# hasindu2008/cornetto

Hardware: AMD Instinct MI355X
Metric: Gbases/s scanned (telowin+sdust+boringbits) (higher is better)
Workload: dtype u8/u16 integer

## Files before the change

### cornetto_amd/csrc/sdust_sift.hpp

```cpp
#pragma once

struct SiftArgs {
    const uint8_t *bases;
    const int64_t *ctg_off;
    const int32_t *ctg_len;
    const SdChunk *chunks;
    int32_t n_chunks;
    int32_t T, W;
    uint32_t lds_per_wave;
    uint32_t reg_cap;
    const uint32_t *order;
    uint32_t *walk_out;
    uint32_t *iswalk_out;
    uint32_t *counter;
    int32_t thr, lmin;
    int32_t abl;
    int32_t dp_min;
    int32_t l2_skip;
};

#ifndef SIFT_WPB
#define SIFT_WPB 1
#endif
constexpr int SIFT_NCTR = 64;
constexpr int SIFT_PAD = 16;
#ifndef SIFT_K
#define SIFT_K 16
#endif
constexpr int SIFT_LS = SIFT_K - 1;
constexpr int SIFT_FIXED = 1024 + 512;
__host__ __device__ constexpr uint32_t sift_lds_bytes(uint32_t cap) { return (SIFT_FIXED + cap / 4 + 2 * (SIFT_PAD + cap) + 16 + 15) / 16 * 16; }


__device__ __forceinline__ uint32_t sd_codes4(uint32_t word)
{
    const uint32_t y = word & 0xDFDFDFDFu, idx = y & 0x07070707u;
    const uint32_t code = __builtin_amdgcn_perm(0x02000003u, 0x01000000u, idx);
    const uint32_t d = y ^ __builtin_amdgcn_perm(0x47FFFF54u, 0x43FF41FFu, idx);
    const uint32_t nz = ((d & 0x7F7F7F7Fu) + 0x7F7F7F7Fu) | d;
    return code | ((nz >> 5) & 0x04040404u);
}
__device__ __forceinline__ uint32_t sd_words4(uint32_t cn, uint32_t pcn)
{
    const uint32_t y1 = __builtin_amdgcn_alignbyte(cn, pcn, 3);
    const uint32_t y2 = __builtin_amdgcn_alignbyte(cn, pcn, 2);
    const uint32_t t = (cn & 0x03030303u) | ((y1 & 0x03030303u) << 2) | ((y2 & 0x03030303u) << 4);
    return t | (((cn | y1 | y2) & 0x04040404u) << 4);
}

__device__ __forceinline__ int sd_mbcnt64(unsigned long long m)
{
    return (int)__builtin_amdgcn_mbcnt_hi((uint32_t)(m >> 32), __builtin_amdgcn_mbcnt_lo((uint32_t)m, 0u));
}
__device__ __forceinline__ int sd_dpp_shr1(int old, int src, bool zero_fill)
{
    return zero_fill ? __builtin_amdgcn_update_dpp(0, src, 0x138, 0xF, 0xF, true) : __builtin_amdgcn_update_dpp(old, src, 0x138, 0xF, 0xF, false);
}

__device__ const uint32_t sd_recip_tab[64] = {0x0u, 0x0u, 0x80000000u, 0x55555556u, 0x40000000u, 0x33333334u, 0x2AAAAAABu, 0x24924925u, 0x20000000u, 0x1C71C71Du, 0x1999999Au, 0x1745D175u, 0x15555556u, 0x13B13B14u, 0x12492493u, 0x11111112u, 0x10000000u, 0xF0F0F10u, 0xE38E38Fu, 0xD79435Fu, 0xCCCCCCDu, 0xC30C30Du, 0xBA2E8BBu, 0xB21642Du, 0xAAAAAABu, 0xA3D70A4u, 0x9D89D8Au, 0x97B425Fu, 0x924924Au, 0x8D3DCB1u, 0x8888889u, 0x8421085u, 0x8000000u, 0x7C1F07Du, 0x7878788u, 0x7507508u, 0x71C71C8u, 0x6EB3E46u, 0x6BCA1B0u, 0x6906907u, 0x6666667u, 0x63E7064u, 0x6186187u, 0x5F417D1u, 0x5D1745Eu, 0x5B05B06u, 0x590B217u, 0x572620Bu, 0x5555556u, 0x539782Au, 0x51EB852u, 0x5050506u, 0x4EC4EC5u, 0x4D4873Fu, 0x4BDA130u, 0x4A7904Bu, 0x4924925u, 0x47DC120u, 0x469EE59u, 0x456C798u, 0x4444445u, 0x4325C54u, 0x4210843u, 0x4104105u};

__device__ __forceinline__ uint32_t sd_scan_max_dpp(uint32_t x)
{
    asm volatile("s_nop 1\n\t"
                 "v_max_u32_dpp %0, %0, %0 row_shr:1 row_mask:0xf bank_mask:0xf\n\ts_nop 1\n\t"
                 "v_max_u32_dpp %0, %0, %0 row_shr:2 row_mask:0xf bank_mask:0xf\n\ts_nop 1\n\t"
                 "v_max_u32_dpp %0, %0, %0 row_shr:4 row_mask:0xf bank_mask:0xf\n\ts_nop 1\n\t"
                 "v_max_u32_dpp %0, %0, %0 row_shr:8 row_mask:0xf bank_mask:0xf\n\ts_nop 1\n\t"
                 "v_max_u32_dpp %0, %0, %0 row_bcast:15 row_mask:0xa bank_mask:0xf\n\ts_nop 1\n\t"
                 "v_max_u32_dpp %0, %0, %0 row_bcast:31 row_mask:0xc bank_mask:0xf\n\ts_nop 1"
                 : "+v"(x));
    return x;
}

__device__ __forceinline__ int sd_wave_find_start(const SdChunk ch, const uint8_t *seq, int W, int lane)
{
    if (ch.start <= 0) return 0;
    const int y = ch.start - 2 * W;
    if (y <= 2) return 0;
    int need = W - 2;
    for (int tile = (y - 1) >> 6, it = 0; tile >= 0 && it < 64; --tile, ++it) {
        const int p = tile * 64 + lane;
        const bool isb = p < y && nt4_code(seq[p]) < 4;
        const unsigned long long b = sd_ballot(isb);
        need -= __popcll(b & (b << 1) & (b << 2));
        if (need <= 0 || tile == 0) return tile * 64;
    }
    return -2;
}

#ifndef SIFT_CHUNK_DEFAULT
#define SIFT_CHUNK_DEFAULT 1792
#endif
constexpr uint32_t SIFT_CAP_DEFAULT = SIFT_CHUNK_DEFAULT + 128;
template <bool STATS, uint32_t CAP = 0>
__global__ __launch_bounds__(64 * SIFT_WPB) __attribute__((amdgpu_waves_per_eu(CAP ? 7 : 6))) void sd_sift(SiftArgs A, SdArgs O)
{
    extern __shared__ __attribute__((aligned(16))) uint8_t sift_lds[];
    const int lane = threadIdx.x & 63;
    const int wave = SIFT_WPB == 1 ? 0 : __builtin_amdgcn_readfirstlane((int)(threadIdx.x >> 6));
    uint8_t *const L = sift_lds + (size_t)wave * (CAP ? sift_lds_bytes(CAP) : A.lds_per_wave);
    uint32_t *const tab = reinterpret_cast<uint32_t *>(L);
    uint16_t *const tl = reinterpret_cast<uint16_t *>(L + 1024);
    uint16_t *const tl2 = tl + 128;
    uint32_t *const sb = reinterpret_cast<uint32_t *>(L + SIFT_FIXED);
    const uint32_t cap = CAP ? CAP : A.reg_cap;
#ifdef CN_DEV
    const int abl = CAP ? 0 : A.abl;
#else
    constexpr int abl = 0;
#endif
    constexpr int STAGE_ROUNDS = CAP ? (int)((CAP + 1023) / 1024) : 4;
    uint32_t *const cb = sb + (cap >> 5);
    uint4 *const col = reinterpret_cast<uint4 *>(tab);
    uint8_t *const wc = L + SIFT_FIXED + cap / 4 + 2 * SIFT_PAD;
    const int T = A.T, W = A.W, CAPW = W - 2;

    const int lo = lane - (CAPW - 1);
    const unsigned long long below = lane ? ~0ull >> (64 - lane) : 0ull;
    const unsigned long long mc = lo > 0 ? below & (~0ull << lo) : below;
    const unsigned long long mp = lo < 0 ? ~0ull << (64 + lo) : 0ull;
    const uint32_t m_a = (uint32_t)mc, m_d = (uint32_t)(mp >> 32), m_m = lane < 32 ? (uint32_t)mp : (uint32_t)(mc >> 32);
    const uint32_t mybit = 1u << (lane & 31);
    uint32_t *const mine0 = tab + (lane < 32 ? 0 : 192), *const mine1 = tab + (lane < 32 ? 64 : 128);
    uint32_t *const tab_mine = mine0;
    const uint32_t *const mid1 = tab + (lane < 32 ? 0 : 128);
    const int thr = A.thr, lmin = A.lmin;
    const int LS = CAPW - 1 < SIFT_LS ? CAPW - 1 : SIFT_LS;
    const bool long_ok = CAPW - 1 > LS;
    unsigned long long st_steps = 0, st_jumps = 0, st_cand = 0, st_trig = 0, st_l1 = 0, st_l2 = 0, st_walk = 0, st_tiles = 0, st_dp = 0, st_g2 = 0, st_g4 = 0, st_g8 = 0;

    struct Meta {
        SdChunk ch;
        int len;
        const uint8_t *seq;
    };
    struct Data {
        uint4 q[2];
        uint32_t pw[2];
    };
    auto meta = [&](int kk) {
        Meta m;
        m.ch = A.chunks[kk];
        m.len = A.ctg_len[m.ch.ctg];
        m.seq = A.bases + A.ctg_off[m.ch.ctg];
        return m;
    };
    auto fetch = [&](const Meta &m) {
        Data d;
        const int rb = m.ch.start - (m.ch.start > 0 ? 128 : 0), rlen = m.ch.end - rb;
#pragma unroll
        for (int it = 0; it < 2; ++it) {
            const int b16 = lane * 16 + it * 1024;
            d.q[it] = make_uint4(0, 0, 0, 0);
            if (b16 < rlen) d.q[it] = *reinterpret_cast<const uint4 *>(m.seq + rb + b16);
        }
        uint32_t first = 0;
        if (rb > 0) first = *reinterpret_cast<const uint32_t *>(m.seq + rb - 4);
        d.pw[0] = (uint32_t)__builtin_amdgcn_update_dpp((int)first, (int)d.q[0].w, 0x138, 0xF, 0xF, false);
        d.pw[1] = (uint32_t)__builtin_amdgcn_update_dpp(rdlane((int)d.q[0].w, 63), (int)d.q[1].w, 0x138, 0xF, 0xF, false);
        return d;
    };

  auto process = [&](const int k, const Meta &M, const Data &D) {
    const SdChunk ch = M.ch;
    const int len = M.len;
    const uint8_t *seq = M.seq;
    const int halo = ch.start > 0 ? 128 : 0;
    const int rb = ch.start - halo;
    const int rlen = ch.end - rb;
    const int ntile = (rlen + 63) >> 6;
    const bool islast = ch.end == len;
    const int rec_from = ch.start;

    tab[lane] = 0;
    tab[64 + lane] = 0;
    tab[128 + lane] = 0;
    tab[192 + lane] = 0;
    for (int i = lane; i < (int)(cap >> 4); i += 64) sb[i] = 0;
    if (lane < SIFT_PAD) reinterpret_cast<uint16_t *>(wc)[lane - SIFT_PAD] = halo ? 0xFF40 : 0x0040;
    bool bad = false;
    bool general = rb <= 0 || rb + ((rlen + 15) & ~15) > len || (abl & 32);
    if (abl & 128) general = false;
    if (!general && !(abl & 128)) {
        uint32_t acc = 0u;
        int lane_s = lane * 16;
        for (int b16 = lane * 16, it = 0; it < STAGE_ROUNDS && b16 < rlen; b16 += 1024, ++it) {
            uint4 q;
            uint32_t pw;
            if (STAGE_ROUNDS <= 2 || it < 2) {
                q = D.q[it];
                pw = D.pw[it];
            } else {
                asm volatile("" : "+v"(lane_s));
                const uint8_t *const g = seq + rb + lane_s + it * 1024;
                q = *reinterpret_cast<const uint4 *>(g);
                pw = *reinterpret_cast<const uint32_t *>(g - 4);
            }
            const uint32_t ipw = pw & 0x07070707u;
            uint32_t pcn = __builtin_amdgcn_perm(0x02000003u, 0x01000000u, ipw);
            acc |= (pw & 0xDFDFDFDFu) ^ __builtin_amdgcn_perm(0x47FFFF54u, 0x43FF41FFu, ipw);
            const uint32_t in[4] = {q.x, q.y, q.z, q.w};
            uint32_t wo[8];
#pragma unroll
            for (int d = 0; d < 4; ++d) {
                const uint32_t idx = in[d] & 0x07070707u;
                const uint32_t cn = __builtin_amdgcn_perm(0x02000003u, 0x01000000u, idx);
                acc |= (in[d] & 0xDFDFDFDFu) ^ __builtin_amdgcn_perm(0x47FFFF54u, 0x43FF41FFu, idx);
                const uint32_t y1 = __builtin_amdgcn_alignbyte(cn, pcn, 3), y2 = __builtin_amdgcn_alignbyte(cn, pcn, 2);
                const uint32_t w4 = cn | y1 << 2 | y2 << 4;
                wo[2 * d] = __builtin_amdgcn_perm(0u, w4, 0x0C010C00u);
                wo[2 * d + 1] = __builtin_amdgcn_perm(0u, w4, 0x0C030C02u);
                pcn = cn;
            }
            uint4 *dst = reinterpret_cast<uint4 *>(wc + 2 * b16);
            dst[0] = make_uint4(wo[0], wo[1], wo[2], wo[3]);
            dst[1] = make_uint4(wo[4], wo[5], wo[6], wo[7]);
        }
        general = sd_any(acc != 0u);
    }
    if (general)
    for (int b16 = lane * 16, it = 0; it < STAGE_ROUNDS && b16 < rlen; b16 += 1024, ++it) {
        const int p0 = rb + b16;
        uint4 q;
        uint32_t pw;
        if (STAGE_ROUNDS <= 2 || it < 2) {
            q = D.q[it];
            pw = D.pw[it];
        } else {
            q = *reinterpret_cast<const uint4 *>(seq + p0);
            pw = *reinterpret_cast<const uint32_t *>(seq + p0 - 4);
        }
        uint32_t pcn = 0x04040404u;
        if (p0 > 0) pcn = sd_codes4(pw);
        const uint32_t in[4] = {q.x, q.y, q.z, q.w};
        uint32_t wo[8];
#pragma unroll
        for (int d = 0; d < 4; ++d) {
            uint32_t cn = sd_codes4(in[d]);
            if (p0 + 4 * d + 4 > len) {
                const int rem = len - (p0 + 4 * d);
                const uint32_t beyond = rem <= 0 ? 0xFFFFFFFFu : 0xFFFFFFFFu << (8 * rem);
                bad = bad || (cn & 0x04040404u & ~beyond) != 0u;
                cn |= 0x04040404u & beyond;
            } else {
                bad = bad || (cn & 0x04040404u) != 0u;
            }
            const uint32_t w4 = sd_words4(cn, pcn);
            wo[2 * d] = __builtin_amdgcn_perm(0u, w4, 0x0C010C00u);
            wo[2 * d + 1] = __builtin_amdgcn_perm(0u, w4, 0x0C030C02u);
            pcn = cn;
        }
        uint4 *dst = reinterpret_cast<uint4 *>(wc + 2 * b16);
        dst[0] = make_uint4(wo[0], wo[1], wo[2], wo[3]);
        dst[1] = make_uint4(wo[4], wo[5], wo[6], wo[7]);
    }
    const bool unclean = sd_any(bad);
    SD_LDS_ORDER();

    int w = 0, r = 0, slot = 0;
    int sv0 = 0;
    bool have_last = false;
    uint32_t last_s = 0, last_f = 0, n_out = 0;
    uint2 *const out = O.out + (size_t)k * O.cap;
    auto emit = [&](int ps, int pf, int tm) {
        if (tm < rec_from) return;
        if (have_last && ps <= (int)last_f) {
            if (pf > (int)last_f) last_f = (uint32_t)pf;
        } else {
            if (have_last) {
                if (n_out < O.cap && lane == 0) out[n_out] = make_uint2(last_s, last_f);
                ++n_out;
            }
            have_last = true;
            last_s = (uint32_t)ps;
            last_f = (uint32_t)pf;
        }
    };
    auto emit_slots = [&](int from, int tm) {
        unsigned long long em = sd_ballot(slot != 0 && lane >= from && lane < CAPW);
        while (em) {
            const int a = 63 - __builtin_clzll(em);
            em &= ~(1ull << a);
            const uint32_t so = (uint32_t)rdlane(slot, a);
            const int s = sv0 - a;
            emit(s, s + (int)(so >> 24) + 3, tm);
        }
    };
    auto push_word = [&](int tw, int amax, bool age_slots) {
        const unsigned long long e = sd_ballot(w == tw) & ~(~1ull << (amax - 1 < 0 ? 0 : amax - 1)) & (amax > 0 ? ~0ull : 0ull);
        r = sd_dpp_shr1(0, r, true) + sd_mbcnt64(e);
        w = sd_dpp_shr1(tw, w, false);
        if (age_slots) slot = sd_dpp_shr1(0, slot, true);
    };
    auto pass = [&](int amax, const int Tl, const uint32_t m_recip) {
        const unsigned long long cm = sd_ballot(__mul24(r, 10) > Tl) & ~(~1ull << amax) & ~1ull;
        if (cm) {
            const bool cand = (cm >> lane) & 1ull;
            if (STATS) ++st_cand;
            uint32_t key_c = 0u;
            if (cand) key_c = lane == 1 ? ((uint32_t)r & 0x7FFu) << 13 : __umulhi(((uint32_t)r & 0x7FFu) << 13, m_recip);
            const uint32_t key_e = (uint32_t)slot & 0xFFFFFFu;
            const uint32_t xs = sd_scan_max_dpp(key_e > key_c ? key_e : key_c);
            const uint32_t sk = (uint32_t)__builtin_amdgcn_update_dpp(0, (int)xs, 0x138, 0xF, 0xF, true);
            const uint32_t km = sk > key_e ? sk : key_e;
            if (cand && key_c >= km) slot = (int)(key_c | ((uint32_t)lane << 24));
        }
    };
    auto finish = [&]() {
        if (have_last) {
            if (n_out < O.cap && lane == 0) out[n_out] = make_uint2(last_s, last_f);
            ++n_out;
        }
        if (lane == 0) {
            O.out_n[k] = n_out;
            if (n_out > O.cap) atomicMax(O.ovf, n_out);
            if (STATS) st_tiles += (unsigned long long)ntile;
        }
    };

    if (unclean) {
        const int Tl = T * lane;
        const uint32_t m_recip = sd_recip_tab[lane];
        if (A.walk_out && lane == 0) {
            A.iswalk_out[k] = 1u;
            A.walk_out[2 + atomicAdd(&A.walk_out[0], 1u)] = (uint32_t)k;
        }
        int u = sd_wave_find_start(ch, seq, W, lane);
        if (u == -2) u = __builtin_amdgcn_readfirstlane(sd_find_start<true>(O, ch, seq));
        if (u < 0) return;
        const int stop = islast ? len + 1 : ch.end;
        int l = 0, size = 0, cv = 4, ctile = -1;
        unsigned t = 0;
        for (int i = u; i < stop; ++i) {
            if ((i >> 6) != ctile) {
                ctile = i >> 6;
                const int p = ctile * 64 + lane;
                cv = p < len ? nt4_code(seq[p]) : 4;
            }
            const int b = rdlane(cv, i & 63);
            if (STATS) ++st_walk;
            if (b < 4) {
                ++l;
                t = (t << 2 | (unsigned)b) & 63u;
                if (l >= 3) {
                    const int start = (l - W > 0 ? l - W : 0) + (i + 1 - l);
                    const bool full = size >= CAPW;
                    const bool moves = l > W;
                    if (full && moves) {
                        const uint32_t so = (uint32_t)rdlane(slot, CAPW - 1);
                        if (so) {
                            const int s = sv0 - (CAPW - 1);
                            emit(s, s + (int)(so >> 24) + 3, i);
                        }
                    }
                    size = full ? CAPW : size + 1;
                    push_word((int)t, size - 1, !full || moves);
                    sv0 = start + size - 1;
                    pass(size - 1, Tl, m_recip);
                }
            } else {
                emit_slots(0, i);
                slot = 0;
                l = 0;
                t = 0;
            }
        }
        finish();
        return;
    }

    typedef __attribute__((address_space(3))) uint32_t lds_u32;
    int ntl = 0, ntl2 = 0;
#ifdef SIFT_L2_ADAPT
    int l2_hot = 0, l2_skipped = 0;
#endif
    auto run_l2 = [&](int nb) {
        const bool on = lane < nb;
        const int o = on ? (int)tl2[lane] : 0;
        bool keep = on;
        if (LS == SIFT_LS) {
            const uint32_t at = (uint32_t)(uintptr_t)(lds_u32 *)wc + 2u * (uint32_t)o - 2u * (uint32_t)(SIFT_K - 1);
            const lds_u32 *const pa = (const lds_u32 *)(uintptr_t)(at & ~3u);
            const uint32_t sh = at & 3u;
            uint32_t k80, ksel1, ksel2, ksel3, kw, kc;
            asm volatile("s_mov_b32 %0, 0x3f3f3f3f\n\ts_mov_b32 %1, 0x01010101\n\ts_mov_b32 %2, 0x02020202\n\ts_mov_b32 %3, 0x03030303\n\t"
                         "s_mov_b32 %4, 0x06040200\n\ts_mov_b32 %5, 0x07050301"
                         : "=s"(k80), "=s"(ksel1), "=s"(ksel2), "=s"(ksel3), "=s"(kw), "=s"(kc));
            uint32_t tt = (uint32_t)T;
            asm volatile("" : "+s"(tt));
            uint32_t Q[4];
#pragma unroll
            for (int q = 0; q < 4; ++q) {
                const uint32_t d0 = pa[2 * q], d1 = pa[2 * q + 1], d2 = pa[2 * q + 2];
                Q[q] = __builtin_amdgcn_perm(__builtin_amdgcn_alignbyte(d2, d1, sh), __builtin_amdgcn_alignbyte(d1, d0, sh), kc);
            }
            uint32_t S = 0;
            unsigned long long pos_m = ~0ull;
#pragma unroll
            for (int a = 0; a < SIFT_K; ++a) {
                const int idx = SIFT_K - 1 - a;
                switch (idx & 3) {
                case 0: asm("v_add_u32_sdwa %0, %1, %0 dst_sel:DWORD dst_unused:UNUSED_PAD src0_sel:BYTE_0 src1_sel:DWORD" : "+v"(S) : "v"(Q[idx >> 2])); break;
                case 1: asm("v_add_u32_sdwa %0, %1, %0 dst_sel:DWORD dst_unused:UNUSED_PAD src0_sel:BYTE_1 src1_sel:DWORD" : "+v"(S) : "v"(Q[idx >> 2])); break;
                case 2: asm("v_add_u32_sdwa %0, %1, %0 dst_sel:DWORD dst_unused:UNUSED_PAD src0_sel:BYTE_2 src1_sel:DWORD" : "+v"(S) : "v"(Q[idx >> 2])); break;
                default: asm("v_add_u32_sdwa %0, %1, %0 dst_sel:DWORD dst_unused:UNUSED_PAD src0_sel:BYTE_3 src1_sel:DWORD" : "+v"(S) : "v"(Q[idx >> 2])); break;
                }
                const uint32_t th = (tt * (uint32_t)(a + 1)) / 10u;
                unsigned long long ok = __builtin_amdgcn_ballot_w64(S > th);
                asm volatile("" : "+s"(ok), "+v"(S));
                pos_m &= ok;
            }
            uint32_t at2 = at & ~3u;
            asm volatile("" : "+v"(at2), "+s"(pos_m));
            const lds_u32 *const pb = (const lds_u32 *)(uintptr_t)at2;
            uint32_t P[4];
#pragma unroll
            for (int q = 0; q < 4; ++q) {
                const uint32_t d0 = pb[2 * q], d1 = pb[2 * q + 1], d2 = pb[2 * q + 2];
                P[q] = __builtin_amdgcn_perm(__builtin_amdgcn_alignbyte(d2, d1, sh), __builtin_amdgcn_alignbyte(d1, d0, sh), kw);
            }
            const uint32_t seen = (P[0] | P[1] | P[2] | P[3]) & 0xC0C0C0C0u;
            uint32_t ne = 0;
            unsigned long long sc_m = 0ull;
#pragma unroll
            for (int a = 1; a < SIFT_K; ++a) {
                const int idx = SIFT_K - 1 - a, qi = idx >> 2, bj = idx & 3;
                const uint32_t rep = __builtin_amdgcn_perm(P[qi], P[qi], bj == 0 ? 0u : bj == 1 ? ksel1 : bj == 2 ? ksel2 : ksel3);
#pragma unroll
                for (int q = qi; q < 4; ++q) {
                    if (q == qi && bj == 3) continue;
                    const uint32_t m = q == qi ? 0x40404040u << (8 * (bj + 1)) : 0x40404040u;
                    const uint32_t u = (P[q] ^ rep) + k80;
                    ne += (uint32_t)__builtin_popcount(u & m);
                }
                const int lim = a * (a + 1) / 2 - (int)((tt * (uint32_t)a) / 10u);
                unsigned long long hit = __builtin_amdgcn_ballot_w64((int)ne < lim);
                asm volatile("" : "+s"(hit), "+v"(ne), "+v"(P[0]), "+v"(P[1]), "+v"(P[2]), "+v"(P[3]));
                sc_m |= hit;
            }
            const bool sc = (sc_m >> lane) & 1ull, pos = (pos_m >> lane) & 1ull;
            keep = on && (seen != 0u || sc || (pos && long_ok));
        }
        if (STATS) st_l2 += (unsigned long long)__popcll(sd_ballot(keep));
#ifdef SIFT_L2_ADAPT
        if (nb == 64) {
            const int kept = __popcll(sd_ballot(keep));
            l2_hot = kept >= SIFT_L2_ADAPT ? (l2_hot < 2 ? l2_hot + 1 : 2) : 0;
            l2_skipped = 0;
        }
#endif
        if (keep) (void)__hip_atomic_fetch_or(&sb[o >> 5], 1u << (o & 31), __ATOMIC_RELAXED, __HIP_MEMORY_SCOPE_WORKGROUP);
    };
    auto run_l1 = [&](int nb) {
        const bool on = lane < nb;
        const int o = on ? (int)tl[lane] : 0;
        const uint8_t *const p = wc + 2 * o;
        int d = 0, dmin = 0x7fffffff;
        if (lmin == 4) {
            uint32_t tt = (uint32_t)T;
            asm volatile("" : "+s"(tt));
            const uint32_t c0 = p[1], c1 = p[-1], c2 = p[-3], c3 = p[-5];
            const uint32_t s1 = c0 + c1, s2 = s1 + c2, s3 = s2 + c3;
            dmin = ((c0 > tt / 10u) & (s1 > (2u * tt) / 10u) & (s2 > (3u * tt) / 10u) & (s3 > (4u * tt) / 10u)) ? 1 : 0;
        } else {
            for (int j = 0; j < lmin; ++j) {
                d += 10 * (int)p[1 - 2 * j] - T;
                dmin = d < dmin ? d : dmin;
            }
        }
        const bool ok = on && dmin > 0;
        const unsigned long long m = sd_ballot(ok);
#ifdef SIFT_L2_ADAPT
        const bool hot = l2_hot >= 2 && __popcll(m) >= 16;
        if (hot && ++l2_skipped >= 12) l2_hot = 1;
        if (__popcll(m) >= A.l2_skip || hot) {
#else
        if (__popcll(m) >= A.l2_skip) {
#endif
            if (STATS) st_l1 += (unsigned long long)__popcll(m);
            if (STATS) st_l2 += (unsigned long long)__popcll(m);
            if (ok) (void)__hip_atomic_fetch_or(&sb[o >> 5], 1u << (o & 31), __ATOMIC_RELAXED, __HIP_MEMORY_SCOPE_WORKGROUP);
        } else if (m) {
            if (STATS) st_l1 += (unsigned long long)__popcll(m);
            if (ok) tl2[ntl2 + sd_mbcnt64(m)] = (uint16_t)o;
            ntl2 += __popcll(m);
            SD_LDS_ORDER();
            if (ntl2 >= 64) {
                run_l2(64);
                const uint16_t mv = tl2[64 + lane];
                SD_LDS_ORDER();
                tl2[lane] = mv;
                ntl2 -= 64;
                SD_LDS_ORDER();
            }
        }
    };

    uint8_t *pq = wc + 2 * lane;
    const uint32_t tab_a = (uint32_t)(uintptr_t)(lds_u32 *)tab, mine0_a = (uint32_t)(uintptr_t)(lds_u32 *)mine0, mine1_a = (uint32_t)(uintptr_t)(lds_u32 *)mine1,
                   mid1_a = (uint32_t)(uintptr_t)(lds_u32 *)mid1;
    auto lds_at = [](uint32_t wi, uint32_t base) __attribute__((always_inline)) {
        uint32_t a;
        asm("v_lshl_add_u32 %0, %1, 2, %2" : "=v"(a) : "v"(wi), "v"(base));
        return (lds_u32 *)(uintptr_t)a;
    };
    uint32_t wv_ahead = pq[0];
    auto tile = [&](auto par_c, auto general_c, auto only_c, const int q) __attribute__((always_inline)) {
        constexpr int PAR = decltype(par_c)::value;
        constexpr bool GENERAL = decltype(general_c)::value, TABLE_ONLY = decltype(only_c)::value;
        constexpr int A_AT = PAR ? 64 : 0, D_AT = PAR ? 192 : 128, M_AT = PAR ? 0 : 64;
        constexpr int Z0 = PAR ? 0 : 64, Z1 = PAR ? 192 : 128;
        constexpr bool CHECK = GENERAL || TABLE_ONLY;
        const uint32_t wv = wv_ahead;
        wv_ahead = pq[128];
        asm("" : "+v"(wv_ahead));
        const bool valid = !CHECK || (wv < 64u && q * 64 + lane < rlen);
        const uint32_t wi = CHECK ? wv & 63u : wv;
        lds_u32 *const t_mine = lds_at(wi, PAR ? mine1_a : mine0_a), *const t_all = lds_at(wi, tab_a), *const t_mid = lds_at(wi, mid1_a);
        if (valid) (void)__hip_atomic_fetch_or(t_mine, mybit, __ATOMIC_RELAXED, __HIP_MEMORY_SCOPE_WORKGROUP);
        SD_LDS_ORDER();
        const uint32_t e_a = t_all[A_AT], e_m = t_mid[M_AT], e_d = t_all[D_AT];
        SD_LDS_ORDER();
        tab[Z0 + lane] = 0;
        tab[Z1 + lane] = 0;
        uint32_t ctu = (uint32_t)__popc(e_a & m_a);
        asm("v_bcnt_u32_b32 %0, %1, %0" : "+v"(ctu) : "v"(e_m & m_m));
        asm("v_bcnt_u32_b32 %0, %1, %0" : "+v"(ctu) : "v"(e_d & m_d));
        const int ct = (int)ctu;
        pq[1] = (uint8_t)(TABLE_ONLY ? 255 : (valid ? ct : 0));
        pq += 128;
        if (!TABLE_ONLY) {
            const bool trig = valid && ct >= thr;
            const unsigned long long m = sd_ballot(trig);
            if (m) {
                if (STATS) st_trig += (unsigned long long)__popcll(m);
                int idx;
                asm("v_cndmask_b32_e64 %0, 64, %1, %2" : "=v"(idx) : "v"(sd_mbcnt64(m)), "s"(m));
                (tl + ntl)[idx] = (uint16_t)(q * 64 + lane);
                ntl += __popcll(m);
                SD_LDS_ORDER();
                if (ntl >= 64) {
                    if (!(abl & 2)) run_l1(64);
                    const uint16_t mv = tl[64 + lane];
                    SD_LDS_ORDER();
                    tl[lane] = mv;
                    ntl -= 64;
                    SD_LDS_ORDER();
                }
            }
        }
    };
    if (!(abl & 4)) {
        using P0 = std::integral_constant<int, 0>;
        using P1 = std::integral_constant<int, 1>;
        int q = 0;
        if (halo) tile(P0{}, std::false_type{}, std::true_type{}, q++);
        else tile(P0{}, std::true_type{}, std::false_type{}, q++);
        for (; q + 1 < ntile - 1; q += 2) {
            tile(P1{}, std::false_type{}, std::false_type{}, q);
            tile(P0{}, std::false_type{}, std::false_type{}, q + 1);
        }
        if (q < ntile - 1) { tile(P1{}, std::false_type{}, std::false_type{}, q); ++q; }
        if (q < ntile) {
            if (q & 1) tile(P1{}, std::true_type{}, std::false_type{}, q);
            else tile(P0{}, std::true_type{}, std::false_type{}, q);
        }
    }
    SD_LDS_ORDER();
    if (ntl > 0 && !(abl & 2)) run_l1(ntl);
    if (ntl2 > 0) run_l2(ntl2);
    if (abl & 1) { finish(); return; }
    SD_LDS_ORDER();

    const int s_lo = ch.start > 0 ? ch.start - W : -0x40000000, s_hi = islast ? 0x7fffffff : ch.end - W;
    int lane_r = lane;
    asm volatile("" : "+v"(lane_r));
    const int Tl = T * lane_r;
    const uint32_t m_recip = sd_recip_tab[lane_r];
    auto mark64 = [&](int o, int nbits) {
        const uint32_t d = (uint32_t)o >> 5, b = (uint32_t)o & 31u;
        const unsigned long long mk = nbits >= 64 ? ~0ull : (1ull << nbits) - 1ull;
        const unsigned long long lo64 = mk << b;
        const uint32_t w1 = (uint32_t)(lo64 >> 32), w2 = b ? (uint32_t)(mk >> (64u - b)) : 0u;
        (void)__hip_atomic_fetch_or(&cb[d], (uint32_t)lo64, __ATOMIC_RELAXED, __HIP_MEMORY_SCOPE_WORKGROUP);
        if (w1) (void)__hip_atomic_fetch_or(&cb[d + 1], w1, __ATOMIC_RELAXED, __HIP_MEMORY_SCOPE_WORKGROUP);
        if (w2) (void)__hip_atomic_fetch_or(&cb[d + 2], w2, __ATOMIC_RELAXED, __HIP_MEMORY_SCOPE_WORKGROUP);
    };
    auto mark = [&](int s, int nbits) {
        if (s < s_lo || s >= s_hi) return;
        if (nbits > 64) {
            mark64(s - rb, 64);
            mark64(s - rb + 64, nbits - 64);
        } else {
            mark64(s - rb, nbits);
        }
    };
    auto pass_m = [&](int amax) {
        const unsigned long long cm = sd_ballot(__mul24(r, 10) > Tl) & ~(~1ull << amax) & ~1ull;
        if (cm) {
            const bool cand = (cm >> lane) & 1ull;
            if (STATS) ++st_cand;
            uint32_t key_c = 0u;
            if (cand) key_c = lane == 1 ? ((uint32_t)r & 0x7FFu) << 13 : __umulhi(((uint32_t)r & 0x7FFu) << 13, m_recip);
            const uint32_t key_e = (uint32_t)slot;
            const uint32_t xs = sd_scan_max_dpp(key_e > key_c ? key_e : key_c);
            const uint32_t sk = (uint32_t)__builtin_amdgcn_update_dpp(0, (int)xs, 0x138, 0xF, 0xF, true);
            const uint32_t km = sk > key_e ? sk : key_e;
            if (cand && key_c >= km) {
                slot = (int)key_c;
                mark(sv0 - lane, lane + 3);
            }
        }
    };

    unsigned long long sw = 0;
    if (lane < ntile) sw = (unsigned long long)sb[2 * lane] | (unsigned long long)sb[2 * lane + 1] << 32;
    if (halo) {
        if (lane == 0) sw = 0;
        if (lane == 1) sw &= ~0ull << (66 - W);
    } else if (lane == 0) {
        sw &= ~3ull;
    }
    tab[lane] = 0;
    tab[192 + lane] = 0;
    SD_LDS_ORDER();

    int cur = 0;
    int n_dense = 0;
    bool have = false;
    bool fresh = false;
    int dp_at = -1;
    int wt = 0, wt_tile = -1;
    bool col_dirty = false;
    auto jump = [&](int i) {
        if (col_dirty) {
            tab[lane] = 0;
            tab[192 + lane] = 0;
            col_dirty = false;
            SD_LDS_ORDER();
        }
        const int o = i - rb;
        const int amax = i - 2 < CAPW - 1 ? i - 2 : CAPW - 1;
        if (STATS) ++st_jumps;
        if (have) {
            const int g = i - cur;
            if (g > 0) {
                const int moved = __builtin_amdgcn_ds_bpermute(((lane - g) & 63) << 2, slot);
                slot = (g < CAPW && lane >= g) ? moved : 0;
            }
        } else {
            slot = 0;
        }
        const bool ok = lane <= amax;
        w = ok ? (int)(wc[2 * (o - lane)] & 63u) : 0;
        if (ok) (void)__hip_atomic_fetch_or(&tab_mine[w], mybit, __ATOMIC_RELAXED, __HIP_MEMORY_SCOPE_WORKGROUP);
        SD_LDS_ORDER();
        const unsigned long long e = (unsigned long long)tab[w] | (unsigned long long)tab[192 + w] << 32;
        SD_LDS_ORDER();
        if (ok) tab_mine[w] = 0;
        SD_LDS_ORDER();
        r = wave_scan_add(ok ? sd_mbcnt64(e) : 0);
        cur = i;
        sv0 = i - 2;
        have = true;
        fresh = true;
    };
    auto dp_tile = [&](int t) {
        const int o0 = 64 * t + lane;
        const uint8_t *const pw = wc + 2 * o0;
        const uint32_t w_own = pw[0];
        int c = 0, rr = 0;
        uint32_t B = 1u, lbest = 0u;
        const bool last = lane == 63;
        auto step = [&](const int l, const uint4 cin, const uint4 cl) __attribute__((always_inline)) {
            const uint32_t wv = pw[-2 * l];
            const uint32_t rcp_l = cl.z;
            const int thr_l = (int)cl.w;
            c = __builtin_amdgcn_update_dpp((int)cin.x, c, 0x138, 0xF, 0xF, false) + (wv == w_own ? 1 : 0);
            rr += c;
            const uint32_t kq = __umulhi((uint32_t)rr << 13, rcp_l);
            const uint32_t key = rr > thr_l ? kq : 0u;
            const uint32_t Bn = (uint32_t)__builtin_amdgcn_update_dpp((int)cin.y, (int)B, 0x138, 0xF, 0xF, false);
            const uint32_t mx = B > Bn ? B : Bn;
            lbest = key >= mx ? (uint32_t)l : lbest;
            asm volatile("" : "+v"(lbest));
            B = mx > key ? mx : key;
            SD_LDS_ORDER();
            if (last) *reinterpret_cast<uint2 *>(&col[l]) = make_uint2((uint32_t)c, B);
        };
        uint4 ca = col[0], cb_ = col[1];
        {
            const uint4 cn = col[2];
            const uint32_t wv = pw[-2];
            c = __builtin_amdgcn_update_dpp((int)ca.x, c, 0x138, 0xF, 0xF, false) + (wv == w_own ? 1 : 0);
            rr += c;
            const uint32_t key = rr > (int)cb_.w ? (uint32_t)rr << 13 : 0u;
            const uint32_t Bn = (uint32_t)__builtin_amdgcn_update_dpp((int)ca.y, (int)B, 0x138, 0xF, 0xF, false);
            const uint32_t mx = B > Bn ? B : Bn;
            lbest = key >= mx ? 1u : lbest;
            B = mx > key ? mx : key;
            SD_LDS_ORDER();
            if (last) *reinterpret_cast<uint2 *>(&col[1]) = make_uint2((uint32_t)c, B);
            ca = cb_;
            cb_ = cn;
        }
        int l = 2;
        for (; l + 1 < CAPW; l += 2) {
            step(l, ca, cb_);
            ca = col[l + 1];
            step(l + 1, cb_, ca);
            cb_ = col[l + 2 < 64 ? l + 2 : 63];
        }
        if (l < CAPW) step(l, ca, cb_);
        if (lbest) mark(rb + o0 - 2 - (int)lbest, (int)lbest + 3);
        SD_LDS_ORDER();
        slot = lane >= 1 && lane < CAPW ? (int)col[lane].y : 0;
        slot = slot == 1 ? 0 : slot;
        SD_LDS_ORDER();
    };
    const int dp_t1 = rlen >> 6;
    unsigned long long nzt = sd_ballot(sw != 0ull);
    while (nzt) {
        const int t = __builtin_ctzll(nzt);
        nzt &= nzt - 1;
        unsigned long long m = rdlane64(sw, t);
        if (__popcll(m) >= A.dp_min && t >= 2 && t < dp_t1) {
            const int e = rb + 64 * t - 1;
            if (dp_at != e) {
                if (!(have && fresh && cur == e)) jump(e);
                const int rprev = sd_dpp_shr1(0, r, true);
                int cc;
                asm volatile("v_sub_u32 %0, %1, %2" : "=v"(cc) : "v"(r), "v"(rprev));
                const uint32_t bb = sd_scan_max_dpp((uint32_t)slot);
                col[lane] = make_uint4((uint32_t)cc, bb > 1u ? bb : 1u, m_recip, (uint32_t)(Tl / 10));
                col_dirty = true;
                SD_LDS_ORDER();
            }
            if (lane == 0) *reinterpret_cast<uint2 *>(&col[0]) = make_uint2(0u, 1u);
            SD_LDS_ORDER();
            dp_tile(t);
            if (STATS) ++st_dp;
            n_dense += 64;
            cur = e + 64;
            dp_at = cur;
            have = true;
            fresh = false;
            continue;
        }
        while (m) {
            const int b = __builtin_ctzll(m);
            const int o = 64 * t + b;
            const int i = rb + o;
            if (have && fresh && i - cur == 1) {
                const unsigned long long inv = ~(m >> b);
                const int run = inv ? __builtin_ctzll(inv) : 64 - b;
                m &= run + b >= 64 ? ~(~0ull << b) : ~(~(~0ull << run) << b);
                if (t != wt_tile) {
                    wt_tile = t;
                    wt = wc[2 * (t * 64 + lane)];
                }
                n_dense += run;
                for (int j = 0; j < run; ++j) {
                    if (STATS) ++st_steps;
                    const int ii = i + j;
                    const int amax = ii - 2 < CAPW - 1 ? ii - 2 : CAPW - 1;
                    push_word(rdlane(wt, b + j), amax, true);
                    sv0 = ii - 2;
                    pass_m(amax);
                }
                cur = i + run - 1;
                continue;
            }
            m &= m - 1;
            if (STATS && have && fresh) { if (i - cur <= 2) ++st_g2; else if (i - cur <= 4) ++st_g4; else if (i - cur <= 8) ++st_g8; }
            jump(i);
            pass_m(i - 2 < CAPW - 1 ? i - 2 : CAPW - 1);
        }
    }
    if (A.walk_out && n_dense >= 256 && lane == 0) {
        A.iswalk_out[k] = 1u;
        A.walk_out[2 + atomicAdd(&A.walk_out[0], 1u)] = (uint32_t)k;
    }
    {
        SD_LDS_ORDER();
        const int nd = (rlen + 31) >> 5;
        uint32_t *const row = reinterpret_cast<uint32_t *>(out);
        uint32_t n_s = 0, n_e = 0;
        int carry = 0;
        for (int base = 0; base <= nd; base += 64) {
            const int d = base + lane;
            const uint32_t v = d < nd ? cb[d] : 0u;
            const unsigned long long nz = sd_ballot(v != 0u);
            if (!nz && carry >= 0) {
                carry = 0;
                continue;
            }
            const uint32_t pm = (uint32_t)__builtin_amdgcn_update_dpp(carry, (int)v, 0x138, 0xF, 0xF, false) >> 31;
            const uint32_t sh = (v << 1) | pm;
            uint32_t st = v & ~sh, en = ~v & sh;
            const int ns = __popc(st), ne = __popc(en);
            const int xs = wave_scan_add(ns), xe = wave_scan_add(ne);
            uint32_t is = n_s + (uint32_t)(xs - ns), ie = n_e + (uint32_t)(xe - ne);
            while (st) {
                const int b = __builtin_ctz(st);
                st &= st - 1;
                if (is < O.cap) row[2 * is] = (uint32_t)(rb + 32 * d + b);
                ++is;
            }
            while (en) {
                const int b = __builtin_ctz(en);
                en &= en - 1;
                if (ie < O.cap) row[2 * ie + 1] = (uint32_t)(rb + 32 * d + b);
                ++ie;
            }
            n_s += (uint32_t)rdlane(xs, 63);
            n_e += (uint32_t)rdlane(xe, 63);
            carry = rdlane((int)v, 63);
        }
        if (lane == 0) {
            O.out_n[k] = n_s;
            if (n_s > O.cap) atomicMax(O.ovf, n_s);
            if (STATS) st_tiles += (unsigned long long)ntile;
        }
    }
  };

    int c = (int)((blockIdx.x * SIFT_WPB + wave) % SIFT_NCTR), dry = 0;
    auto ask = [&](int cc) {
        uint32_t v = 0;
        if (lane == 0) v = atomicAdd(&A.counter[cc * 16], 1u);
        return v;
    };
    uint32_t nxt = ask(c);
    for (;;) {
        const long long kk = (long long)__builtin_amdgcn_readfirstlane((int)nxt) * SIFT_NCTR + c;
        if (kk >= A.n_chunks) {
            static_assert(SIFT_NCTR == 64, "one lane per counter");
            if (dry < 2 * SIFT_NCTR) {
                const uint32_t seen = __hip_atomic_load(&A.counter[lane * 16], __ATOMIC_RELAXED, __HIP_MEMORY_SCOPE_AGENT);
                const long long left = (long long)A.n_chunks - lane;
                const unsigned long long open = sd_ballot(left > 0 && (long long)seen < (left + SIFT_NCTR - 1) / SIFT_NCTR);
                if (!open) break;
                ++dry;
                const int from = c + 1 == SIFT_NCTR ? 0 : c + 1;
                const unsigned long long rot = from ? (open >> from) | (open << (SIFT_NCTR - from)) : open;
                c = (from + __builtin_ctzll(rot)) & (SIFT_NCTR - 1);
                nxt = ask(c);
                continue;
            }
            if (++dry >= 3 * SIFT_NCTR) break;
            c = c + 1 == SIFT_NCTR ? 0 : c + 1;
            nxt = ask(c);
            continue;
        }
        dry = 0;
        nxt = ask(c);
        const int ko = A.order ? __builtin_amdgcn_readfirstlane((int)A.order[kk]) : (int)kk;
        const Meta m = meta(ko);
        process(ko, m, fetch(m));
    }
    if (STATS && O.stats && lane == 0) {
        atomicAdd(&O.stats[0], st_steps);
        atomicAdd(&O.stats[1], st_jumps);
        atomicAdd(&O.stats[2], st_cand);
        atomicAdd(&O.stats[3], st_trig);
        atomicAdd(&O.stats[4], st_l1);
        atomicAdd(&O.stats[5], st_l2);
        atomicAdd(&O.stats[6], st_tiles);
        atomicAdd(&O.stats[7], st_walk);
        atomicAdd(&O.stats[8], st_dp);
        atomicAdd(&O.stats[9], st_g2);
        atomicAdd(&O.stats[10], st_g4);
        atomicAdd(&O.stats[11], st_g8);
    }
}
```

Before: 483.7.

## Split interleaved word/count LDS buffer into separate word and count planes

Replaces the interleaved 2-byte-per-base LDS layout (word byte plus count byte) with two contiguous byte planes: one for words and one for counts, offset by a fixed plane distance. Staging now writes a single 16-byte store per lane instead of two and drops the perm-based byte interleaving. Readers in the long/short sift, DP tile, jump and dense paths switch to unit-stride addressing, and the L1 check loads four counts with one aligned dword plus alignbyte. The cost is the static_assert requiring CAP%64 alignment, and the count-plane offset arithmetic has to be exactly right in every reader.

```diff
diff --git a/cornetto_amd/csrc/sdust_sift.hpp b/cornetto_amd/csrc/sdust_sift.hpp
--- a/cornetto_amd/csrc/sdust_sift.hpp
+++ b/cornetto_amd/csrc/sdust_sift.hpp
@@ -112,7 +112,10 @@
     constexpr int STAGE_ROUNDS = CAP ? (int)((CAP + 1023) / 1024) : 4;
     uint32_t *const cb = sb + (cap >> 5);
     uint4 *const col = reinterpret_cast<uint4 *>(tab);
-    uint8_t *const wc = L + SIFT_FIXED + cap / 4 + 2 * SIFT_PAD;
+    uint8_t *const wds = L + SIFT_FIXED + cap / 4 + SIFT_PAD;
+    static_assert(CAP % 64 == 0 && SIFT_PAD % 16 == 0, "planes: 16-byte aligned words, dword-aligned distance");
+    const uint32_t plane = SIFT_PAD + cap;
+    uint8_t *const cts = wds + plane;
     const int T = A.T, W = A.W, CAPW = W - 2;
 
     const int lo = lane - (CAPW - 1);
@@ -177,7 +180,10 @@
     tab[128 + lane] = 0;
     tab[192 + lane] = 0;
     for (int i = lane; i < (int)(cap >> 4); i += 64) sb[i] = 0;
-    if (lane < SIFT_PAD) reinterpret_cast<uint16_t *>(wc)[lane - SIFT_PAD] = halo ? 0xFF40 : 0x0040;
+    if (lane < SIFT_PAD / 4) {
+        reinterpret_cast<uint32_t *>(wds - SIFT_PAD)[lane] = 0x40404040u;
+        reinterpret_cast<uint32_t *>(cts - SIFT_PAD)[lane] = halo ? 0xFFFFFFFFu : 0u;
+    }
     bool bad = false;
     bool general = rb <= 0 || rb + ((rlen + 15) & ~15) > len || (abl & 32);
     if (abl & 128) general = false;
@@ -200,21 +206,17 @@
             uint32_t pcn = __builtin_amdgcn_perm(0x02000003u, 0x01000000u, ipw);
             acc |= (pw & 0xDFDFDFDFu) ^ __builtin_amdgcn_perm(0x47FFFF54u, 0x43FF41FFu, ipw);
             const uint32_t in[4] = {q.x, q.y, q.z, q.w};
-            uint32_t wo[8];
+            uint32_t wo[4];
 #pragma unroll
             for (int d = 0; d < 4; ++d) {
                 const uint32_t idx = in[d] & 0x07070707u;
                 const uint32_t cn = __builtin_amdgcn_perm(0x02000003u, 0x01000000u, idx);
                 acc |= (in[d] & 0xDFDFDFDFu) ^ __builtin_amdgcn_perm(0x47FFFF54u, 0x43FF41FFu, idx);
                 const uint32_t y1 = __builtin_amdgcn_alignbyte(cn, pcn, 3), y2 = __builtin_amdgcn_alignbyte(cn, pcn, 2);
-                const uint32_t w4 = cn | y1 << 2 | y2 << 4;
-                wo[2 * d] = __builtin_amdgcn_perm(0u, w4, 0x0C010C00u);
-                wo[2 * d + 1] = __builtin_amdgcn_perm(0u, w4, 0x0C030C02u);
+                wo[d] = cn | y1 << 2 | y2 << 4;
                 pcn = cn;
             }
-            uint4 *dst = reinterpret_cast<uint4 *>(wc + 2 * b16);
-            dst[0] = make_uint4(wo[0], wo[1], wo[2], wo[3]);
-            dst[1] = make_uint4(wo[4], wo[5], wo[6], wo[7]);
+            *reinterpret_cast<uint4 *>(wds + b16) = make_uint4(wo[0], wo[1], wo[2], wo[3]);
         }
         general = sd_any(acc != 0u);
     }
@@ -233,7 +235,7 @@
         uint32_t pcn = 0x04040404u;
         if (p0 > 0) pcn = sd_codes4(pw);
         const uint32_t in[4] = {q.x, q.y, q.z, q.w};
-        uint32_t wo[8];
+        uint32_t wo[4];
 #pragma unroll
         for (int d = 0; d < 4; ++d) {
             uint32_t cn = sd_codes4(in[d]);
@@ -245,14 +247,10 @@
             } else {
                 bad = bad || (cn & 0x04040404u) != 0u;
             }
-            const uint32_t w4 = sd_words4(cn, pcn);
-            wo[2 * d] = __builtin_amdgcn_perm(0u, w4, 0x0C010C00u);
-            wo[2 * d + 1] = __builtin_amdgcn_perm(0u, w4, 0x0C030C02u);
+            wo[d] = sd_words4(cn, pcn);
             pcn = cn;
         }
-        uint4 *dst = reinterpret_cast<uint4 *>(wc + 2 * b16);
-        dst[0] = make_uint4(wo[0], wo[1], wo[2], wo[3]);
-        dst[1] = make_uint4(wo[4], wo[5], wo[6], wo[7]);
+        *reinterpret_cast<uint4 *>(wds + b16) = make_uint4(wo[0], wo[1], wo[2], wo[3]);
     }
     const bool unclean = sd_any(bad);
     SD_LDS_ORDER();
@@ -379,20 +377,21 @@
         const int o = on ? (int)tl2[lane] : 0;
         bool keep = on;
         if (LS == SIFT_LS) {
-            const uint32_t at = (uint32_t)(uintptr_t)(lds_u32 *)wc + 2u * (uint32_t)o - 2u * (uint32_t)(SIFT_K - 1);
-            const lds_u32 *const pa = (const lds_u32 *)(uintptr_t)(at & ~3u);
+            const uint32_t at = (uint32_t)(uintptr_t)(lds_u32 *)wds + (uint32_t)o - (uint32_t)(SIFT_K - 1);
+            const lds_u32 *const pa = (const lds_u32 *)(uintptr_t)(at & ~3u) + plane / 4;
             const uint32_t sh = at & 3u;
-            uint32_t k80, ksel1, ksel2, ksel3, kw, kc;
-            asm volatile("s_mov_b32 %0, 0x3f3f3f3f\n\ts_mov_b32 %1, 0x01010101\n\ts_mov_b32 %2, 0x02020202\n\ts_mov_b32 %3, 0x03030303\n\t"
-                         "s_mov_b32 %4, 0x06040200\n\ts_mov_b32 %5, 0x07050301"
-                         : "=s"(k80), "=s"(ksel1), "=s"(ksel2), "=s"(ksel3), "=s"(kw), "=s"(kc));
+            uint32_t k80, ksel1, ksel2, ksel3;
+            asm volatile("s_mov_b32 %0, 0x3f3f3f3f\n\ts_mov_b32 %1, 0x01010101\n\ts_mov_b32 %2, 0x02020202\n\ts_mov_b32 %3, 0x03030303"
+                         : "=s"(k80), "=s"(ksel1), "=s"(ksel2), "=s"(ksel3));
             uint32_t tt = (uint32_t)T;
             asm volatile("" : "+s"(tt));
             uint32_t Q[4];
-#pragma unroll
-            for (int q = 0; q < 4; ++q) {
-                const uint32_t d0 = pa[2 * q], d1 = pa[2 * q + 1], d2 = pa[2 * q + 2];
-                Q[q] = __builtin_amdgcn_perm(__builtin_amdgcn_alignbyte(d2, d1, sh), __builtin_amdgcn_alignbyte(d1, d0, sh), kc);
+            {
+                const uint32_t d0 = pa[0], d1 = pa[1], d2 = pa[2], d3 = pa[3], d4 = pa[4];
+                Q[0] = __builtin_amdgcn_alignbyte(d1, d0, sh);
+                Q[1] = __builtin_amdgcn_alignbyte(d2, d1, sh);
+                Q[2] = __builtin_amdgcn_alignbyte(d3, d2, sh);
+                Q[3] = __builtin_amdgcn_alignbyte(d4, d3, sh);
             }
             uint32_t S = 0;
             unsigned long long pos_m = ~0ull;
@@ -414,10 +413,12 @@
             asm volatile("" : "+v"(at2), "+s"(pos_m));
             const lds_u32 *const pb = (const lds_u32 *)(uintptr_t)at2;
             uint32_t P[4];
-#pragma unroll
-            for (int q = 0; q < 4; ++q) {
-                const uint32_t d0 = pb[2 * q], d1 = pb[2 * q + 1], d2 = pb[2 * q + 2];
-                P[q] = __builtin_amdgcn_perm(__builtin_amdgcn_alignbyte(d2, d1, sh), __builtin_amdgcn_alignbyte(d1, d0, sh), kw);
+            {
+                const uint32_t d0 = pb[0], d1 = pb[1], d2 = pb[2], d3 = pb[3], d4 = pb[4];
+                P[0] = __builtin_amdgcn_alignbyte(d1, d0, sh);
+                P[1] = __builtin_amdgcn_alignbyte(d2, d1, sh);
+                P[2] = __builtin_amdgcn_alignbyte(d3, d2, sh);
+                P[3] = __builtin_amdgcn_alignbyte(d4, d3, sh);
             }
             const uint32_t seen = (P[0] | P[1] | P[2] | P[3]) & 0xC0C0C0C0u;
             uint32_t ne = 0;
@@ -454,17 +455,20 @@
     auto run_l1 = [&](int nb) {
         const bool on = lane < nb;
         const int o = on ? (int)tl[lane] : 0;
-        const uint8_t *const p = wc + 2 * o;
+        const uint8_t *const p = cts + o;
         int d = 0, dmin = 0x7fffffff;
         if (lmin == 4) {
             uint32_t tt = (uint32_t)T;
             asm volatile("" : "+s"(tt));
-            const uint32_t c0 = p[1], c1 = p[-1], c2 = p[-3], c3 = p[-5];
+            const uint32_t a4 = (uint32_t)(uintptr_t)(lds_u32 *)cts + (uint32_t)o - 3u;
+            const lds_u32 *const pc = (const lds_u32 *)(uintptr_t)(a4 & ~3u);
+            const uint32_t c4 = __builtin_amdgcn_alignbyte(pc[1], pc[0], a4 & 3u);
+            const uint32_t c0 = c4 >> 24, c1 = (c4 >> 16) & 255u, c2 = (c4 >> 8) & 255u, c3 = c4 & 255u;
             const uint32_t s1 = c0 + c1, s2 = s1 + c2, s3 = s2 + c3;
             dmin = ((c0 > tt / 10u) & (s1 > (2u * tt) / 10u) & (s2 > (3u * tt) / 10u) & (s3 > (4u * tt) / 10u)) ? 1 : 0;
         } else {
             for (int j = 0; j < lmin; ++j) {
-                d += 10 * (int)p[1 - 2 * j] - T;
+                d += 10 * (int)p[-j] - T;
                 dmin = d < dmin ? d : dmin;
             }
         }
@@ -496,7 +500,7 @@
         }
     };
 
-    uint8_t *pq = wc + 2 * lane;
+    uint8_t *pq = wds + lane;
     const uint32_t tab_a = (uint32_t)(uintptr_t)(lds_u32 *)tab, mine0_a = (uint32_t)(uintptr_t)(lds_u32 *)mine0, mine1_a = (uint32_t)(uintptr_t)(lds_u32 *)mine1,
                    mid1_a = (uint32_t)(uintptr_t)(lds_u32 *)mid1;
     auto lds_at = [](uint32_t wi, uint32_t base) __attribute__((always_inline)) {
@@ -512,7 +516,7 @@
         constexpr int Z0 = PAR ? 0 : 64, Z1 = PAR ? 192 : 128;
         constexpr bool CHECK = GENERAL || TABLE_ONLY;
         const uint32_t wv = wv_ahead;
-        wv_ahead = pq[128];
+        wv_ahead = pq[64];
         asm("" : "+v"(wv_ahead));
         const bool valid = !CHECK || (wv < 64u && q * 64 + lane < rlen);
         const uint32_t wi = CHECK ? wv & 63u : wv;
@@ -527,8 +531,8 @@
         asm("v_bcnt_u32_b32 %0, %1, %0" : "+v"(ctu) : "v"(e_m & m_m));
         asm("v_bcnt_u32_b32 %0, %1, %0" : "+v"(ctu) : "v"(e_d & m_d));
         const int ct = (int)ctu;
-        pq[1] = (uint8_t)(TABLE_ONLY ? 255 : (valid ? ct : 0));
-        pq += 128;
+        pq[plane] = (uint8_t)(TABLE_ONLY ? 255 : (valid ? ct : 0));
+        pq += 64;
         if (!TABLE_ONLY) {
             const bool trig = valid && ct >= thr;
             const unsigned long long m = sd_ballot(trig);
@@ -652,7 +656,7 @@
             slot = 0;
         }
         const bool ok = lane <= amax;
-        w = ok ? (int)(wc[2 * (o - lane)] & 63u) : 0;
+        w = ok ? (int)(wds[o - lane] & 63u) : 0;
         if (ok) (void)__hip_atomic_fetch_or(&tab_mine[w], mybit, __ATOMIC_RELAXED, __HIP_MEMORY_SCOPE_WORKGROUP);
         SD_LDS_ORDER();
         const unsigned long long e = (unsigned long long)tab[w] | (unsigned long long)tab[192 + w] << 32;
@@ -667,13 +671,13 @@
     };
     auto dp_tile = [&](int t) {
         const int o0 = 64 * t + lane;
-        const uint8_t *const pw = wc + 2 * o0;
+        const uint8_t *const pw = wds + o0;
         const uint32_t w_own = pw[0];
         int c = 0, rr = 0;
         uint32_t B = 1u, lbest = 0u;
         const bool last = lane == 63;
         auto step = [&](const int l, const uint4 cin, const uint4 cl) __attribute__((always_inline)) {
-            const uint32_t wv = pw[-2 * l];
+            const uint32_t wv = pw[-l];
             const uint32_t rcp_l = cl.z;
             const int thr_l = (int)cl.w;
             c = __builtin_amdgcn_update_dpp((int)cin.x, c, 0x138, 0xF, 0xF, false) + (wv == w_own ? 1 : 0);
@@ -691,7 +695,7 @@
         uint4 ca = col[0], cb_ = col[1];
         {
             const uint4 cn = col[2];
-            const uint32_t wv = pw[-2];
+            const uint32_t wv = pw[-1];
             c = __builtin_amdgcn_update_dpp((int)ca.x, c, 0x138, 0xF, 0xF, false) + (wv == w_own ? 1 : 0);
             rr += c;
             const uint32_t key = rr > (int)cb_.w ? (uint32_t)rr << 13 : 0u;
@@ -757,7 +761,7 @@
                 m &= run + b >= 64 ? ~(~0ull << b) : ~(~(~0ull << run) << b);
                 if (t != wt_tile) {
                     wt_tile = t;
-                    wt = wc[2 * (t * 64 + lane)];
+                    wt = wds[t * 64 + lane];
                 }
                 n_dense += run;
                 for (int j = 0; j < run; ++j) {
@@ -837,7 +841,9 @@
         if (kk >= A.n_chunks) {
             static_assert(SIFT_NCTR == 64, "one lane per counter");
             if (dry < 2 * SIFT_NCTR) {
-                const uint32_t seen = __hip_atomic_load(&A.counter[lane * 16], __ATOMIC_RELAXED, __HIP_MEMORY_SCOPE_AGENT);
+                int lane_c = lane;
+                asm volatile("" : "+v"(lane_c));
+                const uint32_t seen = __hip_atomic_load(&A.counter[lane_c * 16], __ATOMIC_RELAXED, __HIP_MEMORY_SCOPE_AGENT);
                 const long long left = (long long)A.n_chunks - lane;
                 const unsigned long long open = sd_ballot(left > 0 && (long long)seen < (left + SIFT_NCTR - 1) / SIFT_NCTR);
                 if (!open) break;
```

New measurement: 507.1, median of 6. 4.8% higher.
